# Z-Zheng/ever

Measured on AMD Instinct MI355X. Metric: 512x512 tiles/sec fwd+bwd, FarSeg-R50, higher is better.
Workload: dtype f32; 1 GPU; FarSeg ResNet-50 FPN (FarSegHead defaults, BCE+dice), 3-band 512x512, batch 16/GPU, fwd+bwd+SGD step, inputs resident in HBM; global_batch=16, parallelism=single

## Files before the change

### ever_amd/_C.py

```python
import ctypes as C
import os

_LIB_PATH = os.path.join(os.path.dirname(os.path.abspath(__file__)), 'lib', 'libever_hip.so')
_LIB_PATH = os.environ.get('EVK_LIB', _LIB_PATH)

c_void_p, c_int, c_i32, c_i64, c_u32, c_f32, c_size_t = (
    C.c_void_p, C.c_int, C.c_int32, C.c_int64, C.c_uint32, C.c_float, C.c_size_t)


class ConvDesc(C.Structure):
    _fields_ = [(n, c_i32) for n in (
        'N', 'H', 'W', 'Cin', 'Ho', 'Wo', 'Cout', 'kh', 'kw',
        'stride_h', 'stride_w', 'pad_h', 'pad_w', 'dil_h', 'dil_w')]


class SplitJob(C.Structure):
    _fields_ = [('w', c_void_p), ('out', c_void_p), ('kind', c_i32), ('arg', c_i32 * 13)]


P = c_void_p
_DP = C.POINTER(ConvDesc)
_JP = C.POINTER(SplitJob)

SIGNATURES = {
# ... 66 lines not shown
                                                 P, c_size_t, P, P]),
    'evk_bn_relu_pool_bwd': (c_int, [P, P, P, P, P, P, P, P, P, P, c_i32, c_i32, c_i32, c_i32, c_i32, P, c_size_t, P, P]),
    'evk_bn_bwd': (c_int, [P, P, P, P, P, P, P, P, P, P, P, c_i64, c_i32, c_u32, c_i32, P, c_size_t, P, P]),
    'evk_stream_fork': (c_int, [P, P]),
    'evk_streams_overlap': (c_int, [P, P, c_i32, P]),
    'evk_bn_relu_dot_plan': (c_int, [c_i64, c_i32, c_i32, C.POINTER(c_i32)]),
    'evk_bn_relu_dot_fwd': (c_int, [P, P, P, P, P, c_i64, c_i32, c_i32, P]),
    'evk_bn_relu_dot_workspace_bytes': (c_size_t, [c_i64, c_i32, c_i32]),
    'evk_bn_relu_dot_bwd': (c_int, [P, P, P, P, P, P, P, P, P, P, P, P, c_i64, c_i32, c_i32, c_u32, P, c_size_t, P, P]),
    'evk_bn_finalize_parts': (c_int, [P, c_i32, c_i32, c_i64, P, P, P, P, c_f32, c_f32, P, P, P, P]),
    'evk_relation_bn_fwd': (c_int, [P, P, P, P, P, P, P, c_i32, c_i32, c_i32, P, P]),
    'evk_relation_bn_parts': (c_i32, [c_i32, c_i32]),
    'evk_relation_bn_workspace_bytes': (c_size_t, [c_i32, c_i32, c_i32]),
    'evk_relation_bn_bwd': (c_int, [P, P, P, P, P, P, P, P, P, P, P, P, c_i32, c_i32, c_i32, P, c_size_t, P]),
    'evk_bn_bwd_from_partials': (c_int, [P, P, P, P, P, P, P, c_i32, P, P, P, c_i64, c_i32, c_u32, c_i32, P, c_size_t, P, P]),
    'evk_bn_bwd_bits': (c_int, [P, P, P, P, P, P, P, P, P, P, P, c_i64, c_i32, c_u32, c_i32, P, c_size_t, P, P, P]),
    'evk_bn_fwd_train_parts_dual': (c_int, [P, P, P, P, P, P, c_f32, c_f32, P, P, P, P, c_f32, c_f32, P, P, P, P, P, c_i64, c_i32,
                                            P, c_i32, P, c_i32, P, c_size_t, P, P, P]),
    'evk_bn_bwd_dual': (c_int, [P, P, P, P, P, P, P, P, P, P, P, P, P, P, P, c_i64, c_i32, c_u32, c_u32, P, c_size_t, P, P, P, P]),
    'evk_bn_bwd_dual_fused': (c_int, [c_u32, c_u32]),
    'evk_relu_fwd': (c_int, [P, P, c_i64, P]),
    'evk_relu_bwd': (c_int, [P, P, P, c_i64, P]),
    'evk_add': (c_int, [P, P, P, c_i64, P]),
    'evk_scale': (c_int, [P, c_f32, P, c_i64, P]),
    'evk_group_weight_expand': (c_int, [P, P, c_i32, c_i32, c_i32, c_i32, P]),
    'evk_group_weight_gather': (c_int, [P, P, c_i32, c_i32, c_i32, c_i32, P]),
    'evk_mul_scale': (c_int, [P, P, c_f32, P, c_i64, P]),
    'evk_gelu_fwd': (c_int, [P, P, c_i64, P]),
    'evk_gelu_bwd': (c_int, [P, P, P, c_i64, P]),
    'evk_maxpool3x3s2_fwd': (c_int, [P, P, P, c_i32, c_i32, c_i32, c_i32, P]),
# ... 149 lines not shown
```

### ever_amd/csrc/bn.hip

```cpp
#include "bn_common.hpp"

namespace evk {

__global__ __launch_bounds__(256) void bn_stats_partial_kernel(const float* __restrict__ x, float* __restrict__ partial,
                                                               int64_t rows, int C, int64_t rows_per_blk, int tpc,
                                                               int rl) {
  __shared__ f32x4 red[2][256];
  const int c4 = C >> 2;
  const int tc = threadIdx.x % tpc, tr = threadIdx.x / tpc;
  const int64_t r0 = (int64_t)blockIdx.x * rows_per_blk;
  const int64_t r1 = min(rows, r0 + rows_per_blk);
  for (int cb = tc; cb < c4; cb += tpc) {
    f32x4 s = {0.f, 0.f, 0.f, 0.f}, q = {0.f, 0.f, 0.f, 0.f};
    const f32x4 pv = *reinterpret_cast<const f32x4*>(x + cb * 4);
    if (tr < rl) {
      int64_t r = r0 + tr;
      const int64_t st = rl;
      for (; r + 3 * st < r1; r += 4 * st) {
        const f32x4 v0 = *reinterpret_cast<const f32x4*>(x + r * C + cb * 4) - pv;
        const f32x4 v1 = *reinterpret_cast<const f32x4*>(x + (r + st) * C + cb * 4) - pv;
        const f32x4 v2 = *reinterpret_cast<const f32x4*>(x + (r + 2 * st) * C + cb * 4) - pv;
        const f32x4 v3 = *reinterpret_cast<const f32x4*>(x + (r + 3 * st) * C + cb * 4) - pv;
        s += (v0 + v1) + (v2 + v3);
        q += (v0 * v0 + v1 * v1) + (v2 * v2 + v3 * v3);
// ... 41 lines not shown

__global__ void bn_eval_coef_kernel(const float* __restrict__ gamma, const float* __restrict__ beta,
                                    const float* __restrict__ rm, const float* __restrict__ rv, float eps, int C,
                                    float* __restrict__ scale_shift, float* __restrict__ save_mean,
                                    float* __restrict__ save_invstd, uint32_t* __restrict__ amax) {
  const int c = blockIdx.x * blockDim.x + threadIdx.x;
  zero_amax(amax);
  if (c >= C) return;
  const float invstd = (float)(1.0 / sqrt((double)rv[c] + (double)eps));
  if (save_mean) save_mean[c] = rm[c];
  if (save_invstd) save_invstd[c] = invstd;
  const float g = gamma ? gamma[c] : 1.f, b = beta ? beta[c] : 0.f;
  const float sc = g * invstd;
  scale_shift[c] = sc;
  scale_shift[C + c] = b - rm[c] * sc;
}

__device__ __forceinline__ int chunk_of(size_t blk_base, int c4) {
  const uint32_t v = (uint32_t)(blk_base % (size_t)c4) + threadIdx.x;
  const uint32_t q = (uint32_t)((float)v * (1.0f / (float)c4));
  int r = (int)(v - q * (uint32_t)c4);
  r = r < 0 ? r + c4 : r;
  return r >= c4 ? r - c4 : r;
}

template <bool PK, bool DUAL>
__global__ __launch_bounds__(256) void bn_apply_kernel(const float* __restrict__ x, const float* __restrict__ residual,
                                                       const float* __restrict__ scale_shift,
                                                       const float* __restrict__ scale_shift_b, float* __restrict__ y,
                                                       size_t n4, int C, int relu, uint32_t* __restrict__ amax,
                                                       uint32_t* __restrict__ relu_bits) {
  const size_t base = (size_t)bn_blk() * 256;
  const size_t i = base + threadIdx.x;
  const bool valid = i < n4;
  f32x4 v = {0.f, 0.f, 0.f, 0.f};
  float pk_inv = 1.f;
  if constexpr (PK) pk_inv = op_scale(amax[0]).inv;
  if (valid) {
// ... 171 lines not shown
  if (!reduce_partials<FC>(partial, nblk, C, c, s, q)) return;
  if (dbeta) dbeta[c] = (float)s;
  if (dgamma) dgamma[c] = (float)q;
  const float g = gamma ? gamma[c] : 1.f;
  const float k0 = g * invstd[c], k1 = train ? (float)(s * inv_rows) : 0.f, k2 = train ? (float)(q * inv_rows) : 0.f;
  coef[c] = k0;
  coef[C + c] = k1;
  coef[2 * C + c] = k2;
  if (pmax) {
    const float bound = fabsf(k0) * (gmax + fabsf(k1) + xmax * fabsf(k2));
    uint32_t bits = __builtin_bit_cast(uint32_t, bound);
    if (bound != bound) bits = 0x7fc00000u;
    if (bits) atomicMax(&amax[0], bits);
  }
}
struct BnBwdFinalSet {
  const float *partial, *gamma, *invstd;
  float *dgamma, *dbeta, *coef;
  int train;
  uint32_t* amax;
  const float* pmax;
};
template <typename Set, int NR>
struct BnFinalSets {
  Set row[NR];
};
template <typename Set, int NR>
__device__ __forceinline__ Set bn_final_row(const BnFinalSets<Set, NR>& sets) {
  if constexpr (NR == 1) return sets.row[0];
  else return blockIdx.y ? sets.row[1] : sets.row[0];
}
template <int NR>
__global__ __launch_bounds__(256) void bn_bwd_final_kernel(BnFinalSets<BnBwdFinalSet, NR> sets, int nblk, int C, double inv_rows) {
  const BnBwdFinalSet s = bn_final_row(sets);
  bn_bwd_final_body<kFinCh>(s.partial, nblk, C, inv_rows, s.gamma, s.invstd, s.dgamma, s.dbeta, s.coef, s.train, s.amax, s.pmax);
}

struct BnDxCoef {
  f32x4 k0, k1, k2, mu, is;
};
__device__ __forceinline__ BnDxCoef bn_dx_coef(const float* __restrict__ coef, const float* __restrict__ mean,
                                               const float* __restrict__ invstd, int C, int c) {
  return {reinterpret_cast<const f32x4*>(coef)[c], reinterpret_cast<const f32x4*>(coef + C)[c],
          reinterpret_cast<const f32x4*>(coef + 2 * C)[c], reinterpret_cast<const f32x4*>(mean)[c],
          reinterpret_cast<const f32x4*>(invstd)[c]};
}
template <bool PK>
__device__ __forceinline__ f32x4 bn_dx_store(const BnDxCoef& k, const f32x4 g, const f32x4 xv, float* __restrict__ dx, size_t i,
                                             float pk_inv) {
  const f32x4 xh = (xv - k.mu) * k.is;
  const f32x4 out = k.k0 * (g - k.k1 - xh * k.k2);
  if constexpr (PK) {
    reinterpret_cast<u32x4*>(dx)[i] = pack_hl4(out, pk_inv);
  } else {
    reinterpret_cast<f32x4*>(dx)[i] = out;
  }
  return out;
}
template <bool PK>
__global__ __launch_bounds__(256) void bn_bwd_apply_kernel(const float* __restrict__ dy, const float* __restrict__ x,
                                                           const float* __restrict__ y, const float* __restrict__ mean,
                                                           const float* __restrict__ invstd,
                                                           const float* __restrict__ coef,
                                                           const float* __restrict__ gamma,
                                                           const float* __restrict__ beta, float* __restrict__ dx,
                                                           size_t n4, int C, int relu, uint32_t* __restrict__ amax,
                                                           const uint32_t* __restrict__ bits = nullptr) {
  const size_t base = (size_t)bn_blk() * 256;
  const size_t i = base + threadIdx.x;
  const bool valid = i < n4;
  f32x4 out = {0.f, 0.f, 0.f, 0.f};
  float pk_inv = 1.f;
  if constexpr (PK) pk_inv = op_scale(amax[0]).inv;
// ... 136 lines not shown
}

static void launch_bn_bwd_final_sets(hipStream_t st, const BnBwdFinalSet& a, const BnBwdFinalSet* b, int nblk, int C,
                                     int64_t rows) {
  const dim3 grid((C + kFinCh - 1) / kFinCh, b ? 2 : 1);
  const double inv_rows = 1.0 / (double)rows;
  if (b) hipLaunchKernelGGL(bn_bwd_final_kernel<2>, grid, dim3(256), 0, st, BnFinalSets<BnBwdFinalSet, 2>{{a, *b}}, nblk, C, inv_rows);
  else hipLaunchKernelGGL(bn_bwd_final_kernel<1>, grid, dim3(256), 0, st, BnFinalSets<BnBwdFinalSet, 1>{{a}}, nblk, C, inv_rows);
}
void launch_bn_bwd_final(hipStream_t st, const float* partial, int nblk, int C, int64_t rows, const float* gamma,
                         const float* invstd, float* dgamma, float* dbeta, float* coef, int train, uint32_t* amax,
                         const float* pmax) {
  const BnBwdFinalSet s = {partial, gamma, invstd, dgamma, dbeta, coef, train ? 1 : 0, amax, pmax};
  launch_bn_bwd_final_sets(st, s, nullptr, nblk, C, rows);
}

static void launch_bn_apply(hipStream_t st, bool pack, const float* x, const float* residual, const float* scale_shift,
                            float* y, int64_t rows, int C, uint32_t flags, uint32_t* amax, uint32_t* relu_bits = nullptr,
                            const float* scale_shift_b = nullptr) {
  const size_t n4 = (size_t)rows * C / 4;
  const int relu = (flags & EVK_BN_RELU) ? 1 : 0;
  auto launch = [&](auto kernel) {
    hipLaunchKernelGGL(kernel, dim3(oneshot_grid(n4)), dim3(256), 0, st, x, residual, scale_shift, scale_shift_b, y, n4, C, relu,
                       amax, relu_bits);
  };
  if (scale_shift_b) launch(bn_apply_kernel<false, true>);
  else if (pack) launch(bn_apply_kernel<true, false>);
  else launch(bn_apply_kernel<false, false>);
}

// ... 441 lines not shown
```

### ever_amd/csrc/bn_common.hpp

```cpp
#pragma once
#include "x3_common.hpp"

namespace evk {

__device__ __forceinline__ unsigned bn_blk() { return gridDim.x - 1u - blockIdx.x; }

__device__ __forceinline__ int bn_fin_group() { return xcd_remap((int)blockIdx.x, (int)gridDim.x); }

__device__ __forceinline__ f32x4 bn_ld(const float* p, size_t i) {
  return __builtin_nontemporal_load(reinterpret_cast<const f32x4*>(p) + i);
}

constexpr int kMaxStatBlocks = 2048;

__device__ __forceinline__ void zero_amax(uint32_t* __restrict__ amax) {
  if (amax && blockIdx.x == 0 && threadIdx.x < kAmaxSlots) amax[threadIdx.x * kAmaxStride] = 0;
}

struct BnPlan {
  int nblk;
  int64_t rows_per_blk;
  int tpc, rl;
};
inline BnPlan bn_plan(int64_t rows, int C, int64_t per_override = 0, int64_t cap_override = 0) {
// ... 11 lines not shown
  int64_t rpb = (rows + nb - 1) / nb;
  rpb = ((rpb + p.rl - 1) / p.rl) * p.rl;
  p.rows_per_blk = rpb;
  p.nblk = (int)((rows + rpb - 1) / rpb);
  return p;
}

inline void bn_quad_split(int64_t rows, const BnPlan& pl, int& nblk, int& qpb) {
  const int quads = (int)(rows / 4);
  qpb = (quads + pl.nblk - 1) / pl.nblk;
  qpb = ((qpb + pl.rl - 1) / pl.rl) * pl.rl;
  nblk = (quads + qpb - 1) / qpb;
}

inline unsigned oneshot_grid(size_t n4) { return (unsigned)((n4 + 255) / 256); }

struct BnWorkspace {
  float *partial, *coef, *pmax;
  static size_t bytes(int C) { return ((size_t)kMaxStatBlocks * 4 * C + 8 * (size_t)C) * sizeof(float); }
  BnWorkspace(void* ws, int C)
      : partial((float*)ws), coef(partial + (size_t)kMaxStatBlocks * 2 * C), pmax(coef + 8 * (size_t)C) {}
};

inline int bn_check(const char* what, int64_t rows, int32_t C, const void* ws, size_t ws_bytes, size_t need) {
  EVK_REQUIRE(rows > 0 && C > 0 && C % 4 == 0 && C <= 2048, EVK_E_UNSUPPORTED, "%s: rows=%lld C=%d", what, (long long)rows,
              C);
  EVK_REQUIRE(!need || (ws && ws_bytes >= need), EVK_E_WORKSPACE, "%s: workspace too small", what);
  return EVK_OK;
}

// ... 105 lines not shown
  for (int o = 32; o > 0; o >>= 1) m = max(m, (uint32_t)__shfl_xor((int)m, o, 64));
  if ((threadIdx.x & 63) == 0) red[threadIdx.x >> 6] = m;
  __syncthreads();
  if (threadIdx.x == 0) {
    const uint32_t t = max(max(red[0], red[1]), max(red[2], red[3]));
    if (t) atomicMax(&amax[(blockIdx.x & (kAmaxSlots - 1)) * kAmaxStride], t);
  }
}

void launch_parts_final(hipStream_t st, const float* parts, int nparts, int C, double rows, const float* gamma,
                        const float* beta, float* running_mean, float* running_var, float momentum, float eps,
                        float* save_mean, float* save_invstd, float* scale_shift, uint32_t* amax, int pack);
void launch_bn_bwd_final(hipStream_t st, const float* partial, int nblk, int C, int64_t rows, const float* gamma,
                         const float* invstd, float* dgamma, float* dbeta, float* coef, int train, uint32_t* amax,
                         const float* pmax);

}
```

### ever_amd/csrc/relation.hip

```cpp
#include "stream_common.hpp"

namespace evk {

__device__ __forceinline__ f32x4 bn_relu4(const f32x4 z, const f32x4 sc, const f32x4 sh) {
  f32x4 y = z * sc + sh;
  y.x = fmaxf(y.x, 0.f); y.y = fmaxf(y.y, 0.f); y.z = fmaxf(y.z, 0.f); y.w = fmaxf(y.w, 0.f);
  return y;
}
template <bool BN>
__device__ __forceinline__ f32x4 relation_act(const float* __restrict__ z, const float* __restrict__ ss, int C, int cb) {
  const f32x4 v = *reinterpret_cast<const f32x4*>(z + cb * 4);
  if (!BN) return v;
  return bn_relu4(v, *reinterpret_cast<const f32x4*>(ss + cb * 4), *reinterpret_cast<const f32x4*>(ss + C + cb * 4));
}
template <bool BN>
__global__ __launch_bounds__(256) void relation_fwd_kernel(const float* __restrict__ scene, const float* __restrict__ zc,
                                                           const float* __restrict__ ssc, const float* __restrict__ zf,
                                                           const float* __restrict__ ssf, float* __restrict__ out,
                                                           float* __restrict__ r, int N, int HW, int C,
                                                           uint32_t* __restrict__ amax) {
  const int c4 = C >> 2;
  const int lane = threadIdx.x & 63;
  const size_t npix = (size_t)N * HW;
  const size_t wstride = (size_t)gridDim.x * 4;
// ... 69 lines not shown
  __shared__ double red[32][8];
  const int tc = threadIdx.x & 7, tl = threadIdx.x >> 3;
  const int c = blockIdx.x * 8 + tc;
  const int n = blockIdx.y;
  double s = 0.0;
  if (c < C)
    for (int b = tl; b < nblk; b += 32) s += (double)partial[((size_t)n * nblk + b) * C + c];
  red[tl][tc] = s;
  __syncthreads();
  if (tl == 0 && c < C) {
    for (int k = 1; k < 32; ++k) s += red[k][tc];
    dscene[(size_t)n * C + c] = (float)s;
  }
}

template <int NCH>
__global__ __launch_bounds__(256) void relation_bn_bwd_kernel(
    const float* __restrict__ dout, const float* __restrict__ scene, const float* __restrict__ zc,
    const float* __restrict__ ssc, const float* __restrict__ mic, const float* __restrict__ zf, const float* __restrict__ ssf,
    const float* __restrict__ mif, const float* __restrict__ r, float* __restrict__ gc, float* __restrict__ gf,
    float* __restrict__ partial, float* __restrict__ bnp_c, float* __restrict__ bnm_c, float* __restrict__ bnp_f,
    float* __restrict__ bnm_f, int HW, int C, int pix_per_blk, int nblk) {
  extern __shared__ __attribute__((aligned(16))) float sacc[];
  const int c4 = C >> 2;
  const int lane = threadIdx.x & 63, wave = threadIdx.x >> 6;
  const int n = blockIdx.y;
  const int p0 = blockIdx.x * pix_per_blk, p1 = min(HW, p0 + pix_per_blk);
  const float* sc = scene + (size_t)n * C;
  const f32x4 zero4 = {0.f, 0.f, 0.f, 0.f};
  f32x4 acc[NCH][9];
  f32x4 s4[NCH], scc[NCH], shc[NCH], muc[NCH], isc[NCH], scf[NCH], shf[NCH], muf[NCH], isf[NCH];
#pragma unroll
  for (int j = 0; j < NCH; ++j) {
    const int cb = lane + 64 * j;
    const bool ok = cb < c4;
#pragma unroll
    for (int k = 0; k < 9; ++k) acc[j][k] = zero4;
// ... 18 lines not shown
    for (int j = 0; j < NCH; ++j) {
      const int cb = lane + 64 * j;
      const bool ok = cb < c4;
      a[j] = ok ? *reinterpret_cast<const f32x4*>(dout + pix * C + cb * 4) : zero4;
      zfv[j] = ok ? *reinterpret_cast<const f32x4*>(zf + pix * C + cb * 4) : zero4;
      zcv[j] = ok ? *reinterpret_cast<const f32x4*>(zc + pix * C + cb * 4) : zero4;
    }
    float dot = 0.f;
#pragma unroll
    for (int j = 0; j < NCH; ++j) {
      const int cb = lane + 64 * j;
      const f32x4 y = bn_relu4(zfv[j], scf[j], shf[j]);
      dot += a[j].x * y.x + a[j].y * y.y + a[j].z * y.z + a[j].w * y.w;
      f32x4 g = a[j] * rv;
      g.x = y.x > 0.f ? g.x : 0.f; g.y = y.y > 0.f ? g.y : 0.f; g.z = y.z > 0.f ? g.z : 0.f; g.w = y.w > 0.f ? g.w : 0.f;
      if (cb < c4) *reinterpret_cast<f32x4*>(gf + pix * C + cb * 4) = g;
      const f32x4 xh = (zfv[j] - muf[j]) * isf[j];
      acc[j][5] += g;
      acc[j][6] += g * xh;
      amax4(acc[j][7], g);
      amax4(acc[j][8], xh);
    }
    dot = wave_sum(dot);
    const float dz = dot * rv * (1.f - rv);
#pragma unroll
    for (int j = 0; j < NCH; ++j) {
      const int cb = lane + 64 * j;
      const f32x4 y = bn_relu4(zcv[j], scc[j], shc[j]);
      f32x4 g = s4[j] * dz;
      g.x = y.x > 0.f ? g.x : 0.f; g.y = y.y > 0.f ? g.y : 0.f; g.z = y.z > 0.f ? g.z : 0.f; g.w = y.w > 0.f ? g.w : 0.f;
      if (cb < c4) *reinterpret_cast<f32x4*>(gc + pix * C + cb * 4) = g;
      acc[j][0] += y * dz;
      const f32x4 xh = (zcv[j] - muc[j]) * isc[j];
      acc[j][1] += g;
      acc[j][2] += g * xh;
      amax4(acc[j][3], g);
      amax4(acc[j][4], xh);
    }
  }
  float* my = sacc + (size_t)wave * 9 * C;
#pragma unroll
  for (int j = 0; j < NCH; ++j) {
    const int cb = lane + 64 * j;
    if (cb < c4)
#pragma unroll
      for (int k = 0; k < 9; ++k) *reinterpret_cast<f32x4*>(my + (size_t)k * C + cb * 4) = acc[j][k];
// ... 6 lines not shown
    auto fmx = [&](int k) {
      return fmaxf(fmaxf(sacc[k * C + c], sacc[W9 + k * C + c]), fmaxf(sacc[2 * W9 + k * C + c], sacc[3 * W9 + k * C + c]));
    };
    partial[blk * C + c] = fold(0);
    bnp_c[blk * 2 * C + c] = fold(1);
    bnp_c[blk * 2 * C + C + c] = fold(2);
    bnm_c[blk * 2 * C + c] = fmx(3);
    bnm_c[blk * 2 * C + C + c] = fmx(4);
    bnp_f[blk * 2 * C + c] = fold(5);
    bnp_f[blk * 2 * C + C + c] = fold(6);
    bnm_f[blk * 2 * C + c] = fmx(7);
    bnm_f[blk * 2 * C + C + c] = fmx(8);
  }
}

static int relation_blocks(int HW) {
  constexpr int ppb = 64, cap = 256;
  int b = (HW + ppb - 1) / ppb;
  return b > cap ? cap : (b < 1 ? 1 : b);
}

template <typename F>
static int relation_bwd_launch(const char* what, const float* partial, float* dscene, int N, int HW, int C, hipStream_t st,
                               F&& launch) {
  const int nblk = relation_blocks(HW);
  const int ppb = (HW + nblk - 1) / nblk;
  launch(nblk, ppb);
  int rc = check_launch(what);
  if (rc) return rc;
  hipLaunchKernelGGL(relation_dscene_final_kernel, dim3((C + 7) / 8, N), dim3(256), 0, st, partial, dscene, nblk, C);
// ... 13 lines not shown
  return check_launch("relation_fwd");
}
extern "C" int evk_relation_bn_fwd(const float* scene, const float* zc, const float* scale_shift_c, const float* zf,
                                   const float* scale_shift_f, float* out, float* r, int32_t N, int32_t HW, int32_t C,
                                   uint32_t* out_absmax, void* stream) {
  EVK_REQUIRE(scene && zc && scale_shift_c && zf && scale_shift_f && out && r && nhwc4_ok(N, HW, 1, C), EVK_E_INVALID,
              "relation_bn_fwd: bad argument");
  hipLaunchKernelGGL(relation_fwd_kernel<true>, dim3(grid_for((size_t)N * HW, 4, 8192)), dim3(256), 0, (hipStream_t)stream,
                     scene, zc, scale_shift_c, zf, scale_shift_f, out, r, N, HW, C, out_absmax);
  return check_launch("relation_bn_fwd");
}
extern "C" int32_t evk_relation_bn_parts(int32_t N, int32_t HW) { return (int32_t)relation_records(N, HW); }
extern "C" size_t evk_relation_bn_workspace_bytes(int32_t N, int32_t HW, int32_t C) {
  return C > 0 ? relation_records(N, HW) * C * 9 * sizeof(float) : 0;
}
extern "C" int evk_relation_bn_bwd(const float* dout, const float* scene, const float* zc, const float* scale_shift_c,
                                   const float* mean_invstd_c, const float* zf, const float* scale_shift_f,
                                   const float* mean_invstd_f, const float* r, float* dscene, float* gc, float* gf,
                                   int32_t N, int32_t HW, int32_t C, void* workspace, size_t workspace_bytes,
                                   void* stream) {
  EVK_REQUIRE(dout && scene && zc && scale_shift_c && mean_invstd_c && zf && scale_shift_f && mean_invstd_f && r && dscene &&
                  gc && gf,
              EVK_E_INVALID, "relation_bn_bwd: null pointer");
  EVK_REQUIRE(nhwc4_ok(N, HW, 1, C) && C <= 448, EVK_E_UNSUPPORTED, "relation_bn_bwd: C=%d", C);
  EVK_REQUIRE(workspace && workspace_bytes >= evk_relation_bn_workspace_bytes(N, HW, C), EVK_E_WORKSPACE,
              "relation_bn_bwd: workspace too small");
  const size_t nb = relation_records(N, HW);
  float* w = (float*)workspace;
  float* partial = w;
  float* bnp_c = w + nb * C;
  float* bnm_c = w + nb * 3 * C;
  float* bnp_f = w + nb * 5 * C;
  float* bnm_f = w + nb * 7 * C;
  hipStream_t st = (hipStream_t)stream;
  const size_t lds = (size_t)4 * 9 * C * sizeof(float);
  EVK_REQUIRE(lds <= 64 * 1024, EVK_E_UNSUPPORTED, "relation_bn_bwd: C=%d does not fit the LDS", C);
  return relation_bwd_launch("relation_bn_bwd", partial, dscene, N, HW, C, st, [&](int nblk, int ppb) {
    pick<1, 2, 4>((C / 4 + 63) / 64, [&](auto NCH) {
      hipLaunchKernelGGL(relation_bn_bwd_kernel<NCH()>, dim3(nblk, N), dim3(256), lds, st, dout, scene, zc, scale_shift_c,
                         mean_invstd_c, zf, scale_shift_f, mean_invstd_f, r, gc, gf, partial, bnp_c, bnm_c, bnp_f, bnm_f, HW, C,
                         ppb, nblk);
      return 0;
    });
  });
}
extern "C" size_t evk_relation_workspace_bytes(int32_t N, int32_t HW, int32_t C) {
  return C > 0 ? relation_records(N, HW) * C * sizeof(float) : 0;
}
extern "C" int evk_relation_bwd(const float* dout, const float* scene, const float* content, const float* feat,
                                const float* r, float* dscene, float* dcontent, float* dfeat, int32_t N, int32_t HW,
                                int32_t C, void* workspace, size_t workspace_bytes, void* stream) {
  EVK_REQUIRE(dout && scene && content && feat && r && dscene && dcontent && dfeat, EVK_E_INVALID,
              "relation_bwd: null pointer");
  EVK_REQUIRE(nhwc4_ok(N, HW, 1, C) && C <= 4096, EVK_E_UNSUPPORTED, "relation_bwd: C=%d", C);
  EVK_REQUIRE(workspace && workspace_bytes >= evk_relation_workspace_bytes(N, HW, C), EVK_E_WORKSPACE,
              "relation_bwd: workspace too small");
  hipStream_t st = (hipStream_t)stream;
  return relation_bwd_launch("relation_bwd", (const float*)workspace, dscene, N, HW, C, st, [&](int nblk, int ppb) {
    hipLaunchKernelGGL(relation_bwd_kernel, dim3(nblk, N), dim3(256), 4 * C * sizeof(float), st, dout, scene, content, feat, r,
// ... 4 lines not shown
```

### ever_amd/hip/pointwise.py

```python
import ctypes
import os

import torch
from torch.autograd import Function
from torch.autograd.function import once_differentiable

from .. import _C
from . import timing, weight_planes
from .workspace import workspace
from ._base import (
    HipPathError, _AMAX_HANDOFF, _affine_grads, _amax_zeroed, _conv_out, _dx_scale, _hand_scale, _inherit_amax, _note_amax, _ptr,
    _require_cuda, _same_shape_fake, _stream, _take_handoff, _take_parts, _timed_call, as_nhwc, empty_nhwc,
)
from .streams import (
    _note_param_use,
)
from .conv import (
    _weight_ohwi,
)


class _ReluFn(Function):
    @staticmethod
    def forward(ctx, x):
# ... 305 lines not shown
                stats[1, 2].data_ptr(), out.data_ptr(), r.data_ptr(), n, h * w, c, _ptr(abits), st)
        _AMAX_HANDOFF[0] = (abits, False)
        ctx.pack = (bool(len(parts_c) > 2 and parts_c[2]), bool(len(parts_f) > 2 and parts_f[2]))
        ctx.save_for_backward(scene, zc, zf, wc, wf, stats, r)
        ctx.mark_non_differentiable(*[t for t in (rmc, rvc, rmf, rvf) if t is not None])
        return out

    @staticmethod
    @once_differentiable
    def backward(ctx, dout):
        scene, zc, zf, wc, wf, stats, r = ctx.saved_tensors
        n, c, h, w = zc.shape
        rows, dev, st = n * h * w, zc.device, _stream()
        dout = as_nhwc(dout, 'fs_relation.backward')
        lib = _C.load()
        nb = int(lib.evk_relation_bn_parts(n, h * w))
        ws_bytes = lib.evk_relation_bn_workspace_bytes(n, h * w, c)
        ws = torch.empty((ws_bytes // 4,), device=dev, dtype=torch.float32)
        dscene = empty_nhwc(n, c, 1, 1, dev)
        gc, gf = torch.empty_like(zc), torch.empty_like(zf)
        _C.call('evk_relation_bn_bwd', dout.data_ptr(), scene.data_ptr(), zc.data_ptr(), stats[0, 2].data_ptr(),
                stats[0, 0].data_ptr(), zf.data_ptr(), stats[1, 2].data_ptr(), stats[1, 0].data_ptr(), r.data_ptr(),
                dscene.data_ptr(), gc.data_ptr(), gf.data_ptr(), n, h * w, c, ws.data_ptr(), ws_bytes, st)
        coef = workspace(dev, 16 * c * 4)
        grads = []
        for k, (g, z, gamma) in enumerate(((gc, zc, wc), (gf, zf, wf))):
            sums = ws[nb * c * (1 + 4 * k):]
            maxima = ws[nb * c * (3 + 4 * k):]
            abits, pack = _dx_scale(dev, ctx.pack[k])
            dz = torch.empty_like(z)
            dgamma, dbeta = _affine_grads(gamma, c, dev)
            _timed_call('bn', 12.0 * z.numel(), 'evk_bn_bwd_from_partials', g.data_ptr(), z.data_ptr(), _ptr(gamma),
                        stats[k, 0].data_ptr(), stats[k, 1].data_ptr(), sums.data_ptr(), maxima.data_ptr(), nb, dz.data_ptr(),
                        _ptr(dgamma), _ptr(dbeta), rows, c, 2 if pack else 0, 1, coef.data_ptr(), 16 * c * 4, _ptr(abits), st)
            grads.append((_hand_scale(dz, abits, pack), dgamma, dbeta))
        (dzc, dgc, dbc), (dzf, dgf, dbf) = grads
        return dscene, dzc, dzf, dgc, dbc, dgf, dbf, None, None, None, None, None


def fs_relation_bn(scene, zc, zf, bn_c, bn_f):
    pc, pf = getattr(zc, '_evk_bn_parts', None), getattr(zf, '_evk_bn_parts', None)
    if pc is None or pf is None or pc[1] <= 0 or pf[1] <= 0 or zc.shape != zf.shape or zc.shape[1] % 4 or zc.shape[1] > 448:
        return None
    _take_parts(zc)
    _take_parts(zf)
    n, c, h, w = zc.shape
    scene = as_nhwc(scene.reshape(n, c, 1, 1), 'fs_relation.scene')
    weight_planes.note_running_stats_changed()
    _AMAX_HANDOFF[0] = None

    def stat(bn, name):
        return getattr(bn, name) if bn.track_running_stats else None
# ... 126 lines not shown
```

### include/ever_hip.h

```cpp
#ifndef EVER_HIP_H_
#define EVER_HIP_H_

#include <stddef.h>
#include <stdint.h>

#ifdef __cplusplus
extern "C" {
#endif

#define EVK_OK 0
#define EVK_E_INVALID (-1)
#define EVK_E_UNSUPPORTED (-2)
#define EVK_E_LAUNCH (-3)
#define EVK_E_WORKSPACE (-4)

const char* evk_last_error(void);
int evk_abi_version(void);
const char* evk_build_arch(void);

typedef struct evk_conv_desc {
  int32_t N, H, W, Cin;
  int32_t Ho, Wo, Cout;
  int32_t kh, kw;
  int32_t stride_h, stride_w;
// ... 372 lines not shown
                          float* running_mean, float* running_var, float momentum, float eps, float* save_mean,
                          float* save_invstd, float* scale_shift, void* stream);
int evk_relation_bn_fwd(const float* scene, const float* zc, const float* scale_shift_c, const float* zf,
                        const float* scale_shift_f, float* out, float* r, int32_t N, int32_t HW, int32_t C,
                        uint32_t* out_absmax, void* stream);
int32_t evk_relation_bn_parts(int32_t N, int32_t HW);
size_t evk_relation_bn_workspace_bytes(int32_t N, int32_t HW, int32_t C);
int evk_relation_bn_bwd(const float* dout, const float* scene, const float* zc, const float* scale_shift_c,
                        const float* mean_invstd_c, const float* zf, const float* scale_shift_f, const float* mean_invstd_f,
                        const float* r, float* dscene, float* gc, float* gf, int32_t N, int32_t HW, int32_t C, void* workspace,
                        size_t workspace_bytes, void* stream);
int evk_bn_bwd_from_partials(const float* g, const float* x, const float* gamma, const float* save_mean,
                             const float* save_invstd, const float* partial, const float* maxima, int32_t nparts, float* dx,
                             float* dgamma, float* dbeta, int64_t rows, int32_t C, uint32_t flags, int32_t train,
                             void* workspace, size_t workspace_bytes, uint32_t* dx_absmax, void* stream);

int evk_bn_relu_dot_plan(int64_t rows, int32_t C, int32_t K, int32_t* out);
int evk_bn_relu_dot_fwd(const float* z, const float* scale_shift, const float* w, const float* bias, float* out, int64_t rows,
                        int32_t C, int32_t K, void* stream);
size_t evk_bn_relu_dot_workspace_bytes(int64_t rows, int32_t C, int32_t K);
int evk_bn_relu_dot_bwd(const float* dl, const float* z, const float* scale_shift, const float* gamma, const float* save_mean,
                        const float* save_invstd, const float* w, float* dz, float* dgamma, float* dbeta, float* dw,
                        float* dbias, int64_t rows, int32_t C, int32_t K, uint32_t flags, void* workspace,
                        size_t workspace_bytes, uint32_t* dx_absmax, void* stream);

int evk_bn_local_stats(const float* x, double* stats, int64_t rows, int32_t C, void* workspace,
                       size_t workspace_bytes, void* stream);
int evk_bn_apply_stats(const float* x, const float* residual, const float* gamma, const float* beta,
                       const float* mean, const float* invstd, float* y, int64_t rows, int32_t C,
                       uint32_t flags, void* workspace, size_t workspace_bytes, void* stream);
// ... 61 lines not shown
```

Measured before the change: 575.8 tiles/s.

## Fuse FarSeg relation BN backward into reduce plus single dual apply kernel

The relation backward kernel no longer writes the full gradient tensors gc and gf. It stores only a per-pixel dz scalar, and a new fused apply kernel recomputes both masked gradients and both BN dx outputs in one pass. The two BN final reductions also run in one paired launch. This drops two full-size intermediate writes and reads, plus two separate apply launches, in exchange for recomputing the relu masks and reading dout, zc, zf and scene again in the apply kernel.

Result: no change. 578.0 tiles/s, median of 6 (+0.4%).

```diff
diff --git a/ever_amd/_C.py b/ever_amd/_C.py
--- a/ever_amd/_C.py
+++ b/ever_amd/_C.py
@@ -104,6 +104,8 @@
     'evk_relation_bn_workspace_bytes': (c_size_t, [c_i32, c_i32, c_i32]),
     'evk_relation_bn_bwd': (c_int, [P, P, P, P, P, P, P, P, P, P, P, P, c_i32, c_i32, c_i32, P, c_size_t, P]),
     'evk_bn_bwd_from_partials': (c_int, [P, P, P, P, P, P, P, c_i32, P, P, P, c_i64, c_i32, c_u32, c_i32, P, c_size_t, P, P]),
+    'evk_relation_bn_bwd_reduce': (c_int, [P, P, P, P, P, P, P, P, P, P, P, c_i32, c_i32, c_i32, P, c_size_t, P]),
+    'evk_relation_bn_bwd_apply': (c_int, [P] * 19 + [c_i32, c_i32, c_i32, c_u32, c_u32, P, c_size_t, P, P, P]),
     'evk_bn_bwd_bits': (c_int, [P, P, P, P, P, P, P, P, P, P, P, c_i64, c_i32, c_u32, c_i32, P, c_size_t, P, P, P]),
     'evk_bn_fwd_train_parts_dual': (c_int, [P, P, P, P, P, P, c_f32, c_f32, P, P, P, P, c_f32, c_f32, P, P, P, P, P, c_i64, c_i32,
                                             P, c_i32, P, c_i32, P, c_size_t, P, P, P]),
diff --git a/ever_amd/csrc/bn.hip b/ever_amd/csrc/bn.hip
--- a/ever_amd/csrc/bn.hip
+++ b/ever_amd/csrc/bn.hip
@@ -79,14 +79,6 @@
   const float sc = g * invstd;
   scale_shift[c] = sc;
   scale_shift[C + c] = b - rm[c] * sc;
-}
-
-__device__ __forceinline__ int chunk_of(size_t blk_base, int c4) {
-  const uint32_t v = (uint32_t)(blk_base % (size_t)c4) + threadIdx.x;
-  const uint32_t q = (uint32_t)((float)v * (1.0f / (float)c4));
-  int r = (int)(v - q * (uint32_t)c4);
-  r = r < 0 ? r + c4 : r;
-  return r >= c4 ? r - c4 : r;
 }
 
 template <bool PK, bool DUAL>
@@ -288,13 +280,6 @@
     if (bits) atomicMax(&amax[0], bits);
   }
 }
-struct BnBwdFinalSet {
-  const float *partial, *gamma, *invstd;
-  float *dgamma, *dbeta, *coef;
-  int train;
-  uint32_t* amax;
-  const float* pmax;
-};
 template <typename Set, int NR>
 struct BnFinalSets {
   Set row[NR];
@@ -310,27 +295,6 @@
   bn_bwd_final_body<kFinCh>(s.partial, nblk, C, inv_rows, s.gamma, s.invstd, s.dgamma, s.dbeta, s.coef, s.train, s.amax, s.pmax);
 }
 
-struct BnDxCoef {
-  f32x4 k0, k1, k2, mu, is;
-};
-__device__ __forceinline__ BnDxCoef bn_dx_coef(const float* __restrict__ coef, const float* __restrict__ mean,
-                                               const float* __restrict__ invstd, int C, int c) {
-  return {reinterpret_cast<const f32x4*>(coef)[c], reinterpret_cast<const f32x4*>(coef + C)[c],
-          reinterpret_cast<const f32x4*>(coef + 2 * C)[c], reinterpret_cast<const f32x4*>(mean)[c],
-          reinterpret_cast<const f32x4*>(invstd)[c]};
-}
-template <bool PK>
-__device__ __forceinline__ f32x4 bn_dx_store(const BnDxCoef& k, const f32x4 g, const f32x4 xv, float* __restrict__ dx, size_t i,
-                                             float pk_inv) {
-  const f32x4 xh = (xv - k.mu) * k.is;
-  const f32x4 out = k.k0 * (g - k.k1 - xh * k.k2);
-  if constexpr (PK) {
-    reinterpret_cast<u32x4*>(dx)[i] = pack_hl4(out, pk_inv);
-  } else {
-    reinterpret_cast<f32x4*>(dx)[i] = out;
-  }
-  return out;
-}
 template <bool PK>
 __global__ __launch_bounds__(256) void bn_bwd_apply_kernel(const float* __restrict__ dy, const float* __restrict__ x,
                                                            const float* __restrict__ y, const float* __restrict__ mean,
@@ -497,6 +461,9 @@
   const BnBwdFinalSet s = {partial, gamma, invstd, dgamma, dbeta, coef, train ? 1 : 0, amax, pmax};
   launch_bn_bwd_final_sets(st, s, nullptr, nblk, C, rows);
 }
+void launch_bn_bwd_final_pair(hipStream_t st, const BnBwdFinalSet& a, const BnBwdFinalSet& b, int nblk, int C, int64_t rows) {
+  launch_bn_bwd_final_sets(st, a, &b, nblk, C, rows);
+}
 
 static void launch_bn_apply(hipStream_t st, bool pack, const float* x, const float* residual, const float* scale_shift,
                             float* y, int64_t rows, int C, uint32_t flags, uint32_t* amax, uint32_t* relu_bits = nullptr,
diff --git a/ever_amd/csrc/bn_common.hpp b/ever_amd/csrc/bn_common.hpp
--- a/ever_amd/csrc/bn_common.hpp
+++ b/ever_amd/csrc/bn_common.hpp
@@ -49,6 +49,36 @@
 }
 
 inline unsigned oneshot_grid(size_t n4) { return (unsigned)((n4 + 255) / 256); }
+
+__device__ __forceinline__ int chunk_of(size_t blk_base, int c4) {
+  const uint32_t v = (uint32_t)(blk_base % (size_t)c4) + threadIdx.x;
+  const uint32_t q = (uint32_t)((float)v * (1.0f / (float)c4));
+  int r = (int)(v - q * (uint32_t)c4);
+  r = r < 0 ? r + c4 : r;
+  return r >= c4 ? r - c4 : r;
+}
+
+struct BnDxCoef {
+  f32x4 k0, k1, k2, mu, is;
+};
+__device__ __forceinline__ BnDxCoef bn_dx_coef(const float* __restrict__ coef, const float* __restrict__ mean,
+                                               const float* __restrict__ invstd, int C, int c) {
+  return {reinterpret_cast<const f32x4*>(coef)[c], reinterpret_cast<const f32x4*>(coef + C)[c],
+          reinterpret_cast<const f32x4*>(coef + 2 * C)[c], reinterpret_cast<const f32x4*>(mean)[c],
+          reinterpret_cast<const f32x4*>(invstd)[c]};
+}
+template <bool PK>
+__device__ __forceinline__ f32x4 bn_dx_store(const BnDxCoef& k, const f32x4 g, const f32x4 xv, float* __restrict__ dx, size_t i,
+                                             float pk_inv) {
+  const f32x4 xh = (xv - k.mu) * k.is;
+  const f32x4 out = k.k0 * (g - k.k1 - xh * k.k2);
+  if constexpr (PK) {
+    reinterpret_cast<u32x4*>(dx)[i] = pack_hl4(out, pk_inv);
+  } else {
+    reinterpret_cast<f32x4*>(dx)[i] = out;
+  }
+  return out;
+}
 
 struct BnWorkspace {
   float *partial, *coef, *pmax;
@@ -184,5 +214,13 @@
 void launch_bn_bwd_final(hipStream_t st, const float* partial, int nblk, int C, int64_t rows, const float* gamma,
                          const float* invstd, float* dgamma, float* dbeta, float* coef, int train, uint32_t* amax,
                          const float* pmax);
-
-}
+struct BnBwdFinalSet {
+  const float *partial, *gamma, *invstd;
+  float *dgamma, *dbeta, *coef;
+  int train;
+  uint32_t* amax;
+  const float* pmax;
+};
+void launch_bn_bwd_final_pair(hipStream_t st, const BnBwdFinalSet& a, const BnBwdFinalSet& b, int nblk, int C, int64_t rows);
+
+}
diff --git a/ever_amd/csrc/relation.hip b/ever_amd/csrc/relation.hip
--- a/ever_amd/csrc/relation.hip
+++ b/ever_amd/csrc/relation.hip
@@ -1,3 +1,4 @@
+#include "bn_common.hpp"
 #include "stream_common.hpp"
 
 namespace evk {
@@ -107,13 +108,13 @@
   }
 }
 
-template <int NCH>
+template <int NCH, bool STORE_G>
 __global__ __launch_bounds__(256) void relation_bn_bwd_kernel(
     const float* __restrict__ dout, const float* __restrict__ scene, const float* __restrict__ zc,
     const float* __restrict__ ssc, const float* __restrict__ mic, const float* __restrict__ zf, const float* __restrict__ ssf,
     const float* __restrict__ mif, const float* __restrict__ r, float* __restrict__ gc, float* __restrict__ gf,
     float* __restrict__ partial, float* __restrict__ bnp_c, float* __restrict__ bnm_c, float* __restrict__ bnp_f,
-    float* __restrict__ bnm_f, int HW, int C, int pix_per_blk, int nblk) {
+    float* __restrict__ bnm_f, float* __restrict__ dzpix, int HW, int C, int pix_per_blk, int nblk) {
   extern __shared__ __attribute__((aligned(16))) float sacc[];
   const int c4 = C >> 2;
   const int lane = threadIdx.x & 63, wave = threadIdx.x >> 6;
@@ -162,7 +163,8 @@
       dot += a[j].x * y.x + a[j].y * y.y + a[j].z * y.z + a[j].w * y.w;
       f32x4 g = a[j] * rv;
       g.x = y.x > 0.f ? g.x : 0.f; g.y = y.y > 0.f ? g.y : 0.f; g.z = y.z > 0.f ? g.z : 0.f; g.w = y.w > 0.f ? g.w : 0.f;
-      if (cb < c4) *reinterpret_cast<f32x4*>(gf + pix * C + cb * 4) = g;
+      if constexpr (STORE_G)
+        if (cb < c4) *reinterpret_cast<f32x4*>(gf + pix * C + cb * 4) = g;
       const f32x4 xh = (zfv[j] - muf[j]) * isf[j];
       acc[j][5] += g;
       acc[j][6] += g * xh;
@@ -171,13 +173,16 @@
     }
     dot = wave_sum(dot);
     const float dz = dot * rv * (1.f - rv);
+    if constexpr (!STORE_G)
+      if (lane == 0) dzpix[pix] = dz;
 #pragma unroll
     for (int j = 0; j < NCH; ++j) {
       const int cb = lane + 64 * j;
       const f32x4 y = bn_relu4(zcv[j], scc[j], shc[j]);
       f32x4 g = s4[j] * dz;
       g.x = y.x > 0.f ? g.x : 0.f; g.y = y.y > 0.f ? g.y : 0.f; g.z = y.z > 0.f ? g.z : 0.f; g.w = y.w > 0.f ? g.w : 0.f;
-      if (cb < c4) *reinterpret_cast<f32x4*>(gc + pix * C + cb * 4) = g;
+      if constexpr (STORE_G)
+        if (cb < c4) *reinterpret_cast<f32x4*>(gc + pix * C + cb * 4) = g;
       acc[j][0] += y * dz;
       const f32x4 xh = (zcv[j] - muc[j]) * isc[j];
       acc[j][1] += g;
@@ -214,6 +219,51 @@
   }
 }
 
+__device__ __forceinline__ f32x4 mul_rounded(const f32x4 a, const float b) {
+  f32x4 g = a * b;
+  asm volatile("" : "+v"(g.x), "+v"(g.y), "+v"(g.z), "+v"(g.w));
+  return g;
+}
+template <bool PKC, bool PKF>
+__global__ __launch_bounds__(256) __attribute__((amdgpu_waves_per_eu(8))) void relation_bn_bwd_apply_kernel(
+    const float* __restrict__ dout, const float* __restrict__ scene, const float* __restrict__ zc,
+    const float* __restrict__ ssc, const float* __restrict__ mic, const float* __restrict__ coef_c,
+    const float* __restrict__ zf, const float* __restrict__ ssf, const float* __restrict__ mif,
+    const float* __restrict__ coef_f, const float* __restrict__ r, const float* __restrict__ dzpix, float* __restrict__ dzc,
+    float* __restrict__ dzf, size_t n4, int HW, int C, uint32_t* __restrict__ amax_c, uint32_t* __restrict__ amax_f) {
+  const int c4 = C >> 2;
+  const size_t base = (size_t)bn_blk() * 256;
+  const size_t i = base + threadIdx.x;
+  const bool valid = i < n4;
+  f32x4 outc = {0.f, 0.f, 0.f, 0.f}, outf = {0.f, 0.f, 0.f, 0.f};
+  float pk_inv_c = 1.f, pk_inv_f = 1.f;
+  if constexpr (PKC) pk_inv_c = op_scale(amax_c[0]).inv;
+  if constexpr (PKF) pk_inv_f = op_scale(amax_f[0]).inv;
+  if (valid) {
+    const int c = chunk_of(base, c4);
+    const size_t pix0 = base / (size_t)c4;
+    const uint32_t dp = (uint32_t)((float)(threadIdx.x + (uint32_t)(base % (size_t)c4) - (uint32_t)c) * (1.0f / (float)c4) + 0.5f);
+    const size_t pix = pix0 + dp;
+    const size_t n = pix0 / (size_t)HW + ((uint32_t)(pix0 % (size_t)HW) + dp) / (uint32_t)HW;
+    const BnDxCoef kf = bn_dx_coef(coef_f, mif, mif + C, C, c);
+    const BnDxCoef kc = bn_dx_coef(coef_c, mic, mic + C, C, c);
+    const f32x4 a = bn_ld(dout, i);
+    const f32x4 zfv = bn_ld(zf, i);
+    const f32x4 zcv = bn_ld(zc, i);
+    const float rv = r[pix], dz = dzpix[pix];
+    const f32x4 s4 = reinterpret_cast<const f32x4*>(scene + n * C)[c];
+    const f32x4 yf = bn_relu4(zfv, reinterpret_cast<const f32x4*>(ssf)[c], reinterpret_cast<const f32x4*>(ssf + C)[c]);
+    outf = bn_dx_store<PKF>(kf, relu_mask(mul_rounded(a, rv), yf), zfv, dzf, i, pk_inv_f);
+    const f32x4 yc = bn_relu4(zcv, reinterpret_cast<const f32x4*>(ssc)[c], reinterpret_cast<const f32x4*>(ssc + C)[c]);
+    outc = bn_dx_store<PKC>(kc, relu_mask(mul_rounded(s4, dz), yc), zcv, dzc, i, pk_inv_c);
+  }
+  if constexpr (!PKC)
+    if (amax_c) block_absmax(outc, valid, amax_c);
+  if constexpr (!PKC && !PKF) __syncthreads();
+  if constexpr (!PKF)
+    if (amax_f) block_absmax(outf, valid, amax_f);
+}
+
 static int relation_blocks(int HW) {
   constexpr int ppb = 64, cap = 256;
   int b = (HW + ppb - 1) / ppb;
@@ -257,17 +307,17 @@
 extern "C" size_t evk_relation_bn_workspace_bytes(int32_t N, int32_t HW, int32_t C) {
   return C > 0 ? relation_records(N, HW) * C * 9 * sizeof(float) : 0;
 }
-extern "C" int evk_relation_bn_bwd(const float* dout, const float* scene, const float* zc, const float* scale_shift_c,
-                                   const float* mean_invstd_c, const float* zf, const float* scale_shift_f,
-                                   const float* mean_invstd_f, const float* r, float* dscene, float* gc, float* gf,
-                                   int32_t N, int32_t HW, int32_t C, void* workspace, size_t workspace_bytes,
-                                   void* stream) {
+static int relation_bn_bwd_reduce(const char* what, const float* dout, const float* scene, const float* zc,
+                                  const float* scale_shift_c, const float* mean_invstd_c, const float* zf,
+                                  const float* scale_shift_f, const float* mean_invstd_f, const float* r, float* dscene, float* gc,
+                                  float* gf, float* dzpix, int32_t N, int32_t HW, int32_t C, void* workspace,
+                                  size_t workspace_bytes, void* stream) {
   EVK_REQUIRE(dout && scene && zc && scale_shift_c && mean_invstd_c && zf && scale_shift_f && mean_invstd_f && r && dscene &&
-                  gc && gf,
-              EVK_E_INVALID, "relation_bn_bwd: null pointer");
-  EVK_REQUIRE(nhwc4_ok(N, HW, 1, C) && C <= 448, EVK_E_UNSUPPORTED, "relation_bn_bwd: C=%d", C);
+                  (dzpix || (gc && gf)),
+              EVK_E_INVALID, "%s: null pointer", what);
+  EVK_REQUIRE(nhwc4_ok(N, HW, 1, C) && C <= 448, EVK_E_UNSUPPORTED, "%s: C=%d", what, C);
   EVK_REQUIRE(workspace && workspace_bytes >= evk_relation_bn_workspace_bytes(N, HW, C), EVK_E_WORKSPACE,
-              "relation_bn_bwd: workspace too small");
+              "%s: workspace too small", what);
   const size_t nb = relation_records(N, HW);
   float* w = (float*)workspace;
   float* partial = w;
@@ -277,15 +327,74 @@
   float* bnm_f = w + nb * 7 * C;
   hipStream_t st = (hipStream_t)stream;
   const size_t lds = (size_t)4 * 9 * C * sizeof(float);
-  EVK_REQUIRE(lds <= 64 * 1024, EVK_E_UNSUPPORTED, "relation_bn_bwd: C=%d does not fit the LDS", C);
-  return relation_bwd_launch("relation_bn_bwd", partial, dscene, N, HW, C, st, [&](int nblk, int ppb) {
+  EVK_REQUIRE(lds <= 64 * 1024, EVK_E_UNSUPPORTED, "%s: C=%d does not fit the LDS", what, C);
+  return relation_bwd_launch(what, partial, dscene, N, HW, C, st, [&](int nblk, int ppb) {
     pick<1, 2, 4>((C / 4 + 63) / 64, [&](auto NCH) {
-      hipLaunchKernelGGL(relation_bn_bwd_kernel<NCH()>, dim3(nblk, N), dim3(256), lds, st, dout, scene, zc, scale_shift_c,
-                         mean_invstd_c, zf, scale_shift_f, mean_invstd_f, r, gc, gf, partial, bnp_c, bnm_c, bnp_f, bnm_f, HW, C,
-                         ppb, nblk);
+      auto launch = [&](auto kernel) {
+        hipLaunchKernelGGL(kernel, dim3(nblk, N), dim3(256), lds, st, dout, scene, zc, scale_shift_c, mean_invstd_c, zf,
+                           scale_shift_f, mean_invstd_f, r, gc, gf, partial, bnp_c, bnm_c, bnp_f, bnm_f, dzpix, HW, C, ppb, nblk);
+      };
+      if (dzpix) launch(relation_bn_bwd_kernel<NCH(), false>);
+      else launch(relation_bn_bwd_kernel<NCH(), true>);
       return 0;
     });
   });
+}
+extern "C" int evk_relation_bn_bwd(const float* dout, const float* scene, const float* zc, const float* scale_shift_c,
+                                   const float* mean_invstd_c, const float* zf, const float* scale_shift_f,
+                                   const float* mean_invstd_f, const float* r, float* dscene, float* gc, float* gf,
+                                   int32_t N, int32_t HW, int32_t C, void* workspace, size_t workspace_bytes,
+                                   void* stream) {
+  EVK_REQUIRE(gc && gf, EVK_E_INVALID, "relation_bn_bwd: null pointer");
+  return relation_bn_bwd_reduce("relation_bn_bwd", dout, scene, zc, scale_shift_c, mean_invstd_c, zf, scale_shift_f,
+                                mean_invstd_f, r, dscene, gc, gf, nullptr, N, HW, C, workspace, workspace_bytes, stream);
+}
+extern "C" int evk_relation_bn_bwd_reduce(const float* dout, const float* scene, const float* zc, const float* scale_shift_c,
+                                          const float* mean_invstd_c, const float* zf, const float* scale_shift_f,
+                                          const float* mean_invstd_f, const float* r, float* dscene, float* dz, int32_t N,
+                                          int32_t HW, int32_t C, void* workspace, size_t workspace_bytes, void* stream) {
+  EVK_REQUIRE(dz, EVK_E_INVALID, "relation_bn_bwd_reduce: null pointer");
+  return relation_bn_bwd_reduce("relation_bn_bwd_reduce", dout, scene, zc, scale_shift_c, mean_invstd_c, zf, scale_shift_f,
+                                mean_invstd_f, r, dscene, nullptr, nullptr, dz, N, HW, C, workspace, workspace_bytes, stream);
+}
+extern "C" int evk_relation_bn_bwd_apply(const float* dout, const float* scene, const float* zc, const float* scale_shift_c,
+                                         const float* mean_invstd_c, const float* gamma_c, const float* zf,
+                                         const float* scale_shift_f, const float* mean_invstd_f, const float* gamma_f,
+                                         const float* r, const float* dz, const void* records, float* dzc, float* dzf,
+                                         float* dgamma_c, float* dbeta_c, float* dgamma_f, float* dbeta_f, int32_t N, int32_t HW,
+                                         int32_t C, uint32_t flags_c, uint32_t flags_f, void* workspace, size_t workspace_bytes,
+                                         uint32_t* dzc_absmax, uint32_t* dzf_absmax, void* stream) {
+  EVK_REQUIRE(dout && scene && zc && scale_shift_c && mean_invstd_c && zf && scale_shift_f && mean_invstd_f && r && dz &&
+                  records && dzc && dzf,
+              EVK_E_INVALID, "relation_bn_bwd_apply: null pointer");
+  EVK_REQUIRE(nhwc4_ok(N, HW, 1, C) && C <= 448, EVK_E_UNSUPPORTED, "relation_bn_bwd_apply: C=%d", C);
+  EVK_REQUIRE(workspace && workspace_bytes >= (size_t)8 * C * sizeof(float), EVK_E_WORKSPACE,
+              "relation_bn_bwd_apply: workspace too small");
+  const bool pack_c = (flags_c & EVK_BN_PACK_DX) != 0, pack_f = (flags_f & EVK_BN_PACK_DX) != 0;
+  EVK_REQUIRE((!pack_c || dzc_absmax) && (!pack_f || dzf_absmax), EVK_E_INVALID,
+              "relation_bn_bwd_apply: EVK_BN_PACK_DX needs that output's absmax (slots zero on entry)");
+  const size_t nb = relation_records(N, HW);
+  const int64_t rows = (int64_t)N * HW;
+  const float* w = (const float*)records;
+  float* coef_c = (float*)workspace;
+  float* coef_f = coef_c + (size_t)4 * C;
+  hipStream_t st = (hipStream_t)stream;
+  const BnBwdFinalSet fin_c = {w + nb * C, gamma_c, mean_invstd_c + C, dgamma_c, dbeta_c, coef_c, 1, dzc_absmax,
+                               pack_c ? w + nb * 3 * C : nullptr};
+  const BnBwdFinalSet fin_f = {w + nb * 5 * C, gamma_f, mean_invstd_f + C, dgamma_f, dbeta_f, coef_f, 1, dzf_absmax,
+                               pack_f ? w + nb * 7 * C : nullptr};
+  launch_bn_bwd_final_pair(st, fin_c, fin_f, (int)nb, C, rows);
+  int rc = check_launch("bn_bwd_final");
+  if (rc) return rc;
+  const size_t n4 = (size_t)rows * C / 4;
+  auto launch = [&](auto kernel) {
+    hipLaunchKernelGGL(kernel, dim3(oneshot_grid(n4)), dim3(256), 0, st, dout, scene, zc, scale_shift_c, mean_invstd_c,
+                       (const float*)coef_c, zf, scale_shift_f, mean_invstd_f, (const float*)coef_f, r, dz, dzc, dzf, n4, HW, C,
+                       dzc_absmax, dzf_absmax);
+  };
+  if (pack_c) pack_f ? launch(relation_bn_bwd_apply_kernel<true, true>) : launch(relation_bn_bwd_apply_kernel<true, false>);
+  else pack_f ? launch(relation_bn_bwd_apply_kernel<false, true>) : launch(relation_bn_bwd_apply_kernel<false, false>);
+  return check_launch("relation_bn_bwd_apply");
 }
 extern "C" size_t evk_relation_workspace_bytes(int32_t N, int32_t HW, int32_t C) {
   return C > 0 ? relation_records(N, HW) * C * sizeof(float) : 0;
diff --git a/ever_amd/hip/pointwise.py b/ever_amd/hip/pointwise.py
--- a/ever_amd/hip/pointwise.py
+++ b/ever_amd/hip/pointwise.py
@@ -343,28 +343,24 @@
         rows, dev, st = n * h * w, zc.device, _stream()
         dout = as_nhwc(dout, 'fs_relation.backward')
         lib = _C.load()
-        nb = int(lib.evk_relation_bn_parts(n, h * w))
         ws_bytes = lib.evk_relation_bn_workspace_bytes(n, h * w, c)
         ws = torch.empty((ws_bytes // 4,), device=dev, dtype=torch.float32)
         dscene = empty_nhwc(n, c, 1, 1, dev)
-        gc, gf = torch.empty_like(zc), torch.empty_like(zf)
-        _C.call('evk_relation_bn_bwd', dout.data_ptr(), scene.data_ptr(), zc.data_ptr(), stats[0, 2].data_ptr(),
+        dz = torch.empty((rows,), device=dev, dtype=torch.float32)
+        _C.call('evk_relation_bn_bwd_reduce', dout.data_ptr(), scene.data_ptr(), zc.data_ptr(), stats[0, 2].data_ptr(),
                 stats[0, 0].data_ptr(), zf.data_ptr(), stats[1, 2].data_ptr(), stats[1, 0].data_ptr(), r.data_ptr(),
-                dscene.data_ptr(), gc.data_ptr(), gf.data_ptr(), n, h * w, c, ws.data_ptr(), ws_bytes, st)
-        coef = workspace(dev, 16 * c * 4)
-        grads = []
-        for k, (g, z, gamma) in enumerate(((gc, zc, wc), (gf, zf, wf))):
-            sums = ws[nb * c * (1 + 4 * k):]
-            maxima = ws[nb * c * (3 + 4 * k):]
-            abits, pack = _dx_scale(dev, ctx.pack[k])
-            dz = torch.empty_like(z)
-            dgamma, dbeta = _affine_grads(gamma, c, dev)
-            _timed_call('bn', 12.0 * z.numel(), 'evk_bn_bwd_from_partials', g.data_ptr(), z.data_ptr(), _ptr(gamma),
-                        stats[k, 0].data_ptr(), stats[k, 1].data_ptr(), sums.data_ptr(), maxima.data_ptr(), nb, dz.data_ptr(),
-                        _ptr(dgamma), _ptr(dbeta), rows, c, 2 if pack else 0, 1, coef.data_ptr(), 16 * c * 4, _ptr(abits), st)
-            grads.append((_hand_scale(dz, abits, pack), dgamma, dbeta))
-        (dzc, dgc, dbc), (dzf, dgf, dbf) = grads
-        return dscene, dzc, dzf, dgc, dbc, dgf, dbf, None, None, None, None, None
+                dscene.data_ptr(), dz.data_ptr(), n, h * w, c, ws.data_ptr(), ws_bytes, st)
+        coef = workspace(dev, 8 * c * 4)
+        (abits_c, pack_c), (abits_f, pack_f) = _dx_scale(dev, ctx.pack[0]), _dx_scale(dev, ctx.pack[1])
+        dzc, dzf = torch.empty_like(zc), torch.empty_like(zf)
+        (dgc, dbc), (dgf, dbf) = _affine_grads(wc, c, dev), _affine_grads(wf, c, dev)
+        _timed_call('bn', 20.0 * zc.numel(), 'evk_relation_bn_bwd_apply', dout.data_ptr(), scene.data_ptr(), zc.data_ptr(),
+                    stats[0, 2].data_ptr(), stats[0, 0].data_ptr(), _ptr(wc), zf.data_ptr(), stats[1, 2].data_ptr(),
+                    stats[1, 0].data_ptr(), _ptr(wf), r.data_ptr(), dz.data_ptr(), ws.data_ptr(), dzc.data_ptr(), dzf.data_ptr(),
+                    _ptr(dgc), _ptr(dbc), _ptr(dgf), _ptr(dbf), n, h * w, c, 2 if pack_c else 0, 2 if pack_f else 0,
+                    coef.data_ptr(), 8 * c * 4, _ptr(abits_c), _ptr(abits_f), st)
+        return (dscene, _hand_scale(dzc, abits_c, pack_c), _hand_scale(dzf, abits_f, pack_f), dgc, dbc, dgf, dbf,
+                None, None, None, None, None)
 
 
 def fs_relation_bn(scene, zc, zf, bn_c, bn_f):
diff --git a/include/ever_hip.h b/include/ever_hip.h
--- a/include/ever_hip.h
+++ b/include/ever_hip.h
@@ -410,6 +410,16 @@
                              const float* save_invstd, const float* partial, const float* maxima, int32_t nparts, float* dx,
                              float* dgamma, float* dbeta, int64_t rows, int32_t C, uint32_t flags, int32_t train,
                              void* workspace, size_t workspace_bytes, uint32_t* dx_absmax, void* stream);
+int evk_relation_bn_bwd_reduce(const float* dout, const float* scene, const float* zc, const float* scale_shift_c,
+                               const float* mean_invstd_c, const float* zf, const float* scale_shift_f,
+                               const float* mean_invstd_f, const float* r, float* dscene, float* dz, int32_t N, int32_t HW,
+                               int32_t C, void* workspace, size_t workspace_bytes, void* stream);
+int evk_relation_bn_bwd_apply(const float* dout, const float* scene, const float* zc, const float* scale_shift_c,
+                              const float* mean_invstd_c, const float* gamma_c, const float* zf, const float* scale_shift_f,
+                              const float* mean_invstd_f, const float* gamma_f, const float* r, const float* dz,
+                              const void* records, float* dzc, float* dzf, float* dgamma_c, float* dbeta_c, float* dgamma_f,
+                              float* dbeta_f, int32_t N, int32_t HW, int32_t C, uint32_t flags_c, uint32_t flags_f,
+                              void* workspace, size_t workspace_bytes, uint32_t* dzc_absmax, uint32_t* dzf_absmax, void* stream);
 
 int evk_bn_relu_dot_plan(int64_t rows, int32_t C, int32_t K, int32_t* out);
 int evk_bn_relu_dot_fwd(const float* z, const float* scale_shift, const float* w, const float* bias, float* out, int64_t rows,
```
